# yvette256/nerfstudio-thermal

Hardware: AMD Instinct MI355X
Metric: train rays/sec (4096-ray batch, 96 samples/ray) (higher is better)
Workload: dtype f32; 1 GPU; thermal-nerfacto density_mode=shared train step (pixel sampling+raygen+fwd+losses+bwd+allreduce+Adam), 4096 rays/GPU, 256/96 proposal + 48 field samples, hash 16x2^19x2 + 2x(5x2^17x2), 8 cameras (4 RGB + 4 thermal); rays_per_gpu=4096, parallelism=dp1, grad_scaler=device-side (optim.DeviceGradScaler)

## Files before the change

### nerfstudio-thermal_amd/csrc/tn_common.h

```cpp
#pragma once
#include <hip/hip_runtime.h>
#include <stdint.h>
#include <math.h>
#include "../../include/thermal_nerf_hip.h"

#define TN_WAVE 64

void tn_set_error(const char* fmt, ...);
#define TN_REQUIRE(cond, ...)        \
  do {                               \
    if (!(cond)) {                   \
      tn_set_error(__VA_ARGS__);     \
      return TN_EINVAL;              \
    }                                \
  } while (0)
#define TN_CHECK_LAUNCH(name)                                         \
  do {                                                                \
    hipError_t e__ = hipGetLastError();                               \
    if (e__ != hipSuccess) {                                          \
      tn_set_error("%s: %s", name, hipGetErrorString(e__));           \
      return TN_ELAUNCH;                                              \
    }                                                                 \
  } while (0)

static inline hipStream_t tn_s(tn_stream_t s) { return reinterpret_cast<hipStream_t>(s); }

hipStream_t tn_fork(hipStream_t user);
hipStream_t tn_fork_n(hipStream_t user, int idx);
void tn_join_n(hipStream_t user, int idx);
void tn_join(hipStream_t user, hipStream_t companion);
void tn_join_all(hipStream_t user);
__host__ __device__ static inline int64_t tn_cdiv(int64_t a, int64_t b) { return (a + b - 1) / b; }

struct GridK {
  const float2* table;
  float2* grad;
  int L;
  uint32_t mask;
  uint32_t tsize;
  float res[TN_MAX_LEVELS];
  float* nonfinite;
  int grad_zero;
};
static inline GridK make_gridk(const TnGrid& g) {
  GridK k;
  k.table = reinterpret_cast<const float2*>(g.table);
  k.grad = reinterpret_cast<float2*>(g.table_grad);
  k.L = g.num_levels;
  k.tsize = 1u << g.log2_hashmap_size;
  k.mask = k.tsize - 1u;
  for (int i = 0; i < TN_MAX_LEVELS; ++i) k.res[i] = g.res[i];
  k.nonfinite = g.nonfinite_flag;
  k.grad_zero = g.table_grad_is_zero;
  return k;
}

int tn_prop_density_fwd_ex(const TnPropNet* net, const float* origins, const float* directions, const float* e_bins, int64_t N, int32_t S,
                           float* density, float* enc_out, tn_stream_t stream);
int tn_prop_density_bwd_ex(const TnPropNet* net, const float* origins, const float* directions, const float* e_bins, const float* d_density, int64_t N,
                           int32_t S, void* workspace, int64_t workspace_bytes, float* d_origins, float* d_directions, const float* saved_enc,
                           tn_stream_t stream);
int tn_field_fwd_ex(const TnField* field, const float* origins, const float* directions, const int64_t* camera_indices, const float* e_bins, int64_t N, int32_t S,
                    int32_t training, void* workspace, int64_t workspace_bytes, float* density, float* rgb, float* density_pre, int pack_first, void* zero,
                    int64_t zero_bytes, tn_stream_t stream);

int64_t tn_knn_tree_workspace_bytes(int64_t n);
int tn_knn_neighbor_means(const float* points, int64_t n, int32_t nb_neighbors, double* mean, void* workspace, int64_t workspace_bytes,
                          hipStream_t stream);

struct SplatCropK {
  float m[12];
  float h[3];
};
__device__ __forceinline__ bool splat_in_crop(const SplatCropK& c, float x, float y, float z) {
  bool in = true;
#pragma unroll
  for (int a = 0; a < 3; ++a) {
    const float q = __fadd_rn(__fadd_rn(__fadd_rn(__fmul_rn(c.m[4 * a], x), __fmul_rn(c.m[4 * a + 1], y)), __fmul_rn(c.m[4 * a + 2], z)), c.m[4 * a + 3]);
    in = in && fabsf(q) < c.h[a];
  }
  return in;
}
static inline SplatCropK make_cropk(const TnSplatCrop* crop) {
  SplatCropK c;
  for (int i = 0; i < 12; ++i) c.m[i] = crop->world_to_box[i];
  for (int i = 0; i < 3; ++i) c.h[i] = crop->half_extent[i];
  return c;
}

#define TN_PRIME_Y 2654435761u
#define TN_PRIME_Z 805459861u

__device__ __forceinline__ float tn_nan_to_num(float x) {
  if (x != x) return 0.0f;
  if (x > 3.4028234663852886e38f) return 3.4028234663852886e38f;
  if (x < -3.4028234663852886e38f) return -3.4028234663852886e38f;
  return x;
}

__device__ __forceinline__ float tn_spacing(float x) { return x < 1.0f ? x / 2.0f : 1.0f - 1.0f / (2.0f * x); }
__device__ __forceinline__ float tn_spacing_inv(float x) { return x < 0.5f ? 2.0f * x : 1.0f / (2.0f - 2.0f * x); }
__device__ __forceinline__ float tn_s_to_euclid(float x, float s_near, float s_far) {
  return tn_spacing_inv(x * s_far + (1.0f - x) * s_near);
}

__device__ __forceinline__ int64_t tn_div_index(int64_t i, int64_t d, int64_t total) {
  return total < (1ll << 31) ? (int64_t)((uint32_t)i / (uint32_t)d) : i / d;
}

__device__ __forceinline__ void tn_spaced_bins_ray(const float* __restrict__ lin_bins, bool jittered, float jit, float s_near, float s_far, int S,
                                                   float* __restrict__ sb, float* __restrict__ eb, int lane, float* e_keep = nullptr,
                                                   float* s_keep = nullptr) {
#pragma unroll
  for (int k = 0; k <= TN_MAX_SAMPLES / 64; ++k) {
    const int j = lane + 64 * k;
    if (j > S) continue;
    float b = lin_bins[j];
    if (jittered) {
      float lower = (j == 0) ? lin_bins[0] : (lin_bins[j] + lin_bins[j - 1]) / 2.0f;
      float upper = (j == S) ? lin_bins[S] : (lin_bins[j + 1] + lin_bins[j]) / 2.0f;
      b = lower + (upper - lower) * jit;
    }
    const float e = tn_s_to_euclid(b, s_near, s_far);
    sb[j] = b;
    eb[j] = e;
    if (e_keep != nullptr) e_keep[j] = e;
    if (s_keep != nullptr) s_keep[k] = b;
  }
}
__device__ __forceinline__ void tn_spaced_bins_body(const float* __restrict__ lin_bins, const float* __restrict__ jitter,
                                                    const float* __restrict__ nears, const float* __restrict__ fars, int64_t N, int S,
                                                    float* __restrict__ s_bins, float* __restrict__ e_bins, int bid, int nblk) {
  const int lane = threadIdx.x & 63, wpb = blockDim.x >> 6;
  for (int64_t ray = (int64_t)bid * wpb + (threadIdx.x >> 6); ray < N; ray += (int64_t)nblk * wpb) {
    const float s_near = tn_spacing(nears[ray]), s_far = tn_spacing(fars[ray]);
    const float jit = jitter != nullptr ? jitter[ray] : 0.0f;
    tn_spaced_bins_ray(lin_bins, jitter != nullptr, jit, s_near, s_far, S, s_bins + ray * (S + 1), e_bins + ray * (S + 1), lane);
  }
}

struct Contracted {
  float px, py, pz;
  bool sel;
  float wx, wy, wz;
  float mag;
  int amax;
};
__device__ __forceinline__ Contracted tn_contract(float ox, float oy, float oz, float dx, float dy, float dz, float start, float end) {
  Contracted c;
  float se = start + end;
  c.wx = ox + (dx * se) / 2.0f;
  c.wy = oy + (dy * se) / 2.0f;
  c.wz = oz + (dz * se) / 2.0f;
  float ax = fabsf(c.wx), ay = fabsf(c.wy), az = fabsf(c.wz);
  float mag = fmaxf(fmaxf(ax, ay), az);
  c.mag = mag;
  c.amax = (ax >= ay && ax >= az) ? 0 : (ay >= az ? 1 : 2);
  float x = c.wx, y = c.wy, z = c.wz;
  if (!(mag < 1.0f)) {
    float k = 2.0f - (1.0f / mag);
    x = k * (x / mag);
    y = k * (y / mag);
    z = k * (z / mag);
  }
  x = (x + 2.0f) / 4.0f;
  y = (y + 2.0f) / 4.0f;
  z = (z + 2.0f) / 4.0f;
  c.sel = (x > 0.0f) && (x < 1.0f) && (y > 0.0f) && (y < 1.0f) && (z > 0.0f) && (z < 1.0f);
  float m = c.sel ? 1.0f : 0.0f;
  c.px = x * m;
  c.py = y * m;
  c.pz = z * m;
  return c;
}

__device__ __forceinline__ void tn_contract_bwd(const Contracted& c, float gx, float gy, float gz, float& wx, float& wy, float& wz) {
  if (!c.sel) { wx = wy = wz = 0.0f; return; }
  gx *= 0.25f; gy *= 0.25f; gz *= 0.25f;
  if (c.mag < 1.0f) { wx = gx; wy = gy; wz = gz; return; }
  float m = c.mag;
  float s = 2.0f / m - 1.0f / (m * m);
  float t = (-2.0f / (m * m) + 2.0f / (m * m * m));
  float dot = gx * c.wx + gy * c.wy + gz * c.wz;
  wx = s * gx; wy = s * gy; wz = s * gz;
  float xa = c.amax == 0 ? c.wx : (c.amax == 1 ? c.wy : c.wz);
  float extra = dot * t * (xa >= 0.0f ? 1.0f : -1.0f);
  if (c.amax == 0) wx += extra; else if (c.amax == 1) wy += extra; else wz += extra;
}

struct LevelCorners {
  uint32_t idx[8];
  float ox, oy, oz;
};
__device__ __forceinline__ void tn_level_corners(float px, float py, float pz, float res, uint32_t mask, uint32_t level_off, LevelCorners& lc) {
  float sx = px * res, sy = py * res, sz = pz * res;
  float fxf = floorf(sx), fyf = floorf(sy), fzf = floorf(sz);
  uint32_t cx = (uint32_t)(int)ceilf(sx), cy = (uint32_t)(int)ceilf(sy), cz = (uint32_t)(int)ceilf(sz);
  uint32_t fx = (uint32_t)(int)fxf, fy = (uint32_t)(int)fyf, fz = (uint32_t)(int)fzf;
  lc.ox = sx - fxf; lc.oy = sy - fyf; lc.oz = sz - fzf;
  uint32_t hcy = cy * TN_PRIME_Y, hfy = fy * TN_PRIME_Y, hcz = cz * TN_PRIME_Z, hfz = fz * TN_PRIME_Z;
  lc.idx[0] = ((cx ^ hcy ^ hcz) & mask) + level_off;
  lc.idx[1] = ((cx ^ hfy ^ hcz) & mask) + level_off;
  lc.idx[2] = ((fx ^ hfy ^ hcz) & mask) + level_off;
  lc.idx[3] = ((fx ^ hcy ^ hcz) & mask) + level_off;
  lc.idx[4] = ((cx ^ hcy ^ hfz) & mask) + level_off;
  lc.idx[5] = ((cx ^ hfy ^ hfz) & mask) + level_off;
  lc.idx[6] = ((fx ^ hfy ^ hfz) & mask) + level_off;
  lc.idx[7] = ((fx ^ hcy ^ hfz) & mask) + level_off;
}
// ... 203 lines not shown
```

### nerfstudio-thermal_amd/csrc/tn_pipeline.hip

```cpp
#include "tn_common.h"
#include "tn_pose_finish.h"
#include "tn_adam.h"

namespace {
struct EvalWs {
  float *s0, *e0, *d0, *w0, *s1, *e1, *d1, *w1, *s2, *e2, *w2, *rgb_s, *scratch;
  void* field_ws;
  int64_t bytes;
};
EvalWs eval_layout(void* base, int64_t N, int S0, int S1, int S2, int C) {
  EvalWs w;
  char* p = reinterpret_cast<char*>(base);
  int64_t off = 0;
  auto take = [&](int64_t floats) {
    float* r = reinterpret_cast<float*>(p + off);
    off += ((floats * 4 + 255) / 256) * 256;
    return r;
  };
  w.s0 = take(N * (S0 + 1)); w.e0 = take(N * (S0 + 1)); w.d0 = take(N * S0); w.w0 = take(N * S0);
  w.s1 = take(N * (S1 + 1)); w.e1 = take(N * (S1 + 1)); w.d1 = take(N * S1); w.w1 = take(N * S1);
  w.s2 = take(N * (S2 + 1)); w.e2 = take(N * (S2 + 1)); w.w2 = take(N * S2);
  w.rgb_s = take(N * (int64_t)S2 * C);
  w.scratch = take(TN_RENDER_SCRATCH_FLOATS);
  w.field_ws = p + off;
  off += tn_field_workspace_bytes(N * (int64_t)S2, 0);
  w.bytes = off;
  return w;
}
}

extern "C" int64_t tn_render_rays_eval_workspace_bytes(int64_t num_rays, int32_t S0, int32_t S1, int32_t S2, int32_t C) {
  if (num_rays < 0 || S0 < 1 || S1 < 1 || S2 < 1 || S0 > TN_MAX_SAMPLES || S1 > TN_MAX_SAMPLES || S2 > TN_MAX_SAMPLES || C < 1 || C > 4) return TN_EINVAL;
  return eval_layout(nullptr, num_rays, S0, S1, S2, C).bytes;
}

extern "C" int tn_render_rays_eval(const TnPropNet* prop0, const TnPropNet* prop1, const TnField* field, const float* origins,
                                   const float* directions, const int64_t* camera_indices, const float* nears, const float* fars, int64_t N,
                                   int32_t S0, int32_t S1, int32_t S2, float anneal, const float* lin_spaced0, const float* lin_pdf1,
                                   const float* lin_pdf2, void* workspace, int64_t workspace_bytes, float* rgb, float* accumulation, float* depth_median,
                                   float* depth_expected, float* prop_depth0, float* prop_depth1, float* density, float* e_bins_out,
                                   float* rgb_samples_out, tn_stream_t stream) {
  if (N == 0) return TN_OK;
  TN_REQUIRE(prop0 && prop1 && field && origins && directions && camera_indices && nears && fars && lin_spaced0 && lin_pdf1 && lin_pdf2 &&
                 workspace && rgb && density,
             "tn_render_rays_eval: null pointer");
  TN_REQUIRE(N > 0 && S0 >= 1 && S1 >= 1 && S2 >= 1 && S0 <= TN_MAX_SAMPLES && S1 <= TN_MAX_SAMPLES && S2 <= TN_MAX_SAMPLES,
             "tn_render_rays_eval: bad N=%lld S=(%d, %d, %d)", (long long)N, S0, S1, S2);
  TN_REQUIRE(((uintptr_t)workspace % 256) == 0, "tn_render_rays_eval: workspace must be 256-byte aligned");
  const int C = field->num_channels;
  EvalWs w = eval_layout(workspace, N, S0, S1, S2, C);
  TN_REQUIRE(workspace_bytes >= w.bytes, "tn_render_rays_eval: workspace of %lld bytes, tn_render_rays_eval_workspace_bytes = %lld", (long long)workspace_bytes,
             (long long)w.bytes);
  const int64_t field_ws_bytes = tn_field_workspace_bytes(N * (int64_t)S2, 0);
  float* e2 = e_bins_out ? e_bins_out : w.e2;
  float* rgb_s = rgb_samples_out ? rgb_samples_out : w.rgb_s;
  int rc;
  if ((rc = tn_spaced_bins(lin_spaced0, nullptr, nears, fars, N, S0, w.s0, w.e0, stream))) return rc;
  if ((rc = tn_prop_density_fwd(prop0, origins, directions, w.e0, N, S0, w.d0, stream))) return rc;
  if ((rc = tn_weights_resample(w.e0, w.d0, w.s0, S0, anneal, lin_pdf1, nullptr, nears, fars, N, S1, w.w0, prop_depth0, w.s1, w.e1, stream))) return rc;
  if ((rc = tn_prop_density_fwd(prop1, origins, directions, w.e1, N, S1, w.d1, stream))) return rc;
  if ((rc = tn_weights_resample(w.e1, w.d1, w.s1, S1, anneal, lin_pdf2, nullptr, nears, fars, N, S2, w.w1, prop_depth1, w.s2, e2, stream))) return rc;
  if ((rc = tn_field_fwd_ex(field, origins, directions, camera_indices, e2, N, S2, 0, w.field_ws, field_ws_bytes, density, rgb_s, nullptr, 1, nullptr, 0, stream)))
    return rc;
  return tn_render_fwd(e2, density, rgb_s, N, S2, C, 0, w.w2, rgb, accumulation, depth_median, depth_expected, w.scratch, stream);
}

enum {
  TRO_ORIGINS = 0, TRO_DIRECTIONS,
  TRO_S0, TRO_E0, TRO_D0, TRO_W0, TRO_M0,
  TRO_S1, TRO_E1, TRO_D1, TRO_W1, TRO_M1,
  TRO_S2, TRO_E2, TRO_D2, TRO_W2,
  TRO_RGB_SAMPLES, TRO_COMP, TRO_ACC, TRO_DEPTH, TRO_EXPECTED, TRO_SCRATCH,
  TRO_PENC0, TRO_PENC1,
  TRO_END,
  TRO_COUNT
};
static void train_layout(int64_t N, int S0, int S1, int S2, int C, int64_t* off) {
  int64_t o = 0;
  auto take = [&](int slot, int64_t floats) { off[slot] = o; o += (floats + 63) / 64 * 64; };
  take(TRO_ORIGINS, N * 3); take(TRO_DIRECTIONS, N * 3);
  take(TRO_S0, N * (S0 + 1)); take(TRO_E0, N * (S0 + 1)); take(TRO_D0, N * S0); take(TRO_W0, N * S0); take(TRO_M0, N);
  take(TRO_S1, N * (S1 + 1)); take(TRO_E1, N * (S1 + 1)); take(TRO_D1, N * S1); take(TRO_W1, N * S1); take(TRO_M1, N);
  take(TRO_S2, N * (S2 + 1)); take(TRO_E2, N * (S2 + 1)); take(TRO_D2, N * S2); take(TRO_W2, N * S2);
  take(TRO_RGB_SAMPLES, N * (int64_t)S2 * C); take(TRO_COMP, N * C); take(TRO_ACC, N); take(TRO_DEPTH, N); take(TRO_EXPECTED, N);
  take(TRO_SCRATCH, TN_RENDER_SCRATCH_FLOATS);
  take(TRO_PENC0, N * (int64_t)S0 * 10); take(TRO_PENC1, N * (int64_t)S1 * 10);
  off[TRO_END] = o;
}

extern "C" int tn_render_rays_train_layout(int64_t num_rays, int32_t S0, int32_t S1, int32_t S2, int32_t C, int64_t* offsets, int32_t num_offsets) {
  TN_REQUIRE(offsets != nullptr && num_offsets >= TRO_COUNT, "tn_render_rays_train_layout: offsets needs %d entries", (int)TRO_COUNT);
  TN_REQUIRE(num_rays >= 0 && S0 >= 1 && S1 >= 1 && S2 >= 1 && S0 <= TN_MAX_SAMPLES && S1 <= TN_MAX_SAMPLES && S2 <= TN_MAX_SAMPLES && C >= 1 && C <= 4,
             "tn_render_rays_train_layout: bad argument");
  train_layout(num_rays, S0, S1, S2, C, offsets);
  return TN_OK;
}

static int render_rays_train_impl(const TnPropNet* prop0, const TnPropNet* prop1, const TnField* field, const float* pose_adjustment,
                                  const uint8_t* frozen, int32_t num_cameras, const float* origins_in, const float* directions_in,
                                  const int64_t* camera_indices, const float* nears, const float* fars, int64_t N, int32_t S0, int32_t S1,
                                  int32_t S2, float anneal, const float* jitter0, const float* jitter1, const float* jitter2,
                                  const float* lin_spaced0, const float* lin_pdf1, const float* lin_pdf2, void* field_workspace,
                                  int64_t field_workspace_bytes, float* out, void* wait_event_before_field, void* zero_fill, int64_t zero_fill_bytes,
                                  int32_t save_prop_enc, int with_render, int* clip_nblk, tn_stream_t stream, bool sampling_done = false) {
  if (clip_nblk) *clip_nblk = 0;
  if (N == 0) return TN_OK;
  TN_REQUIRE(prop0 && prop1 && field && origins_in && directions_in && camera_indices && nears && fars && lin_spaced0 && lin_pdf1 && lin_pdf2 &&
                 field_workspace && out,
             "tn_render_rays_train: null pointer");
  TN_REQUIRE(N > 0 && S0 >= 1 && S1 >= 1 && S2 >= 1 && S0 <= TN_MAX_SAMPLES && S1 <= TN_MAX_SAMPLES && S2 <= TN_MAX_SAMPLES,
             "tn_render_rays_train: bad N=%lld S=(%d, %d, %d)", (long long)N, S0, S1, S2);
  TN_REQUIRE(((uintptr_t)out % 256) == 0, "tn_render_rays_train: the output buffer must be 256-byte aligned");
  const int C = field->num_channels;
  int64_t off[TRO_COUNT];
  train_layout(N, S0, S1, S2, C, off);
  auto at = [&](int slot) { return out + off[slot]; };
  const float* o = origins_in;
  const float* d = directions_in;
  int rc;
  if (sampling_done) {
    if (pose_adjustment != nullptr) { o = at(TRO_ORIGINS); d = at(TRO_DIRECTIONS); }
  } else {
    if (pose_adjustment != nullptr) {
      TN_REQUIRE(num_cameras >= 1, "tn_render_rays_train: bad num_cameras=%d", num_cameras);
      if ((rc = tn_pose_spaced_bins(pose_adjustment, frozen, camera_indices, origins_in, directions_in, N, num_cameras, at(TRO_ORIGINS), at(TRO_DIRECTIONS),
                                    lin_spaced0, jitter0, nears, fars, S0, at(TRO_S0), at(TRO_E0), stream)))
        return rc;
      o = at(TRO_ORIGINS);
      d = at(TRO_DIRECTIONS);
    } else if ((rc = tn_spaced_bins(lin_spaced0, jitter0, nears, fars, N, S0, at(TRO_S0), at(TRO_E0), stream))) {
      return rc;
    }
    if ((rc = tn_prop_density_fwd_ex(prop0, o, d, at(TRO_E0), N, S0, at(TRO_D0), save_prop_enc ? at(TRO_PENC0) : nullptr, stream))) return rc;
    if ((rc = tn_weights_resample(at(TRO_E0), at(TRO_D0), at(TRO_S0), S0, anneal, lin_pdf1, jitter1, nears, fars, N, S1, at(TRO_W0), at(TRO_M0), at(TRO_S1),
                                  at(TRO_E1), stream)))
      return rc;
    if ((rc = tn_prop_density_fwd_ex(prop1, o, d, at(TRO_E1), N, S1, at(TRO_D1), save_prop_enc ? at(TRO_PENC1) : nullptr, stream))) return rc;
    if ((rc = tn_weights_resample(at(TRO_E1), at(TRO_D1), at(TRO_S1), S1, anneal, lin_pdf2, jitter2, nears, fars, N, S2, at(TRO_W1), at(TRO_M1), at(TRO_S2),
                                  at(TRO_E2), stream)))
      return rc;
  }
  if (wait_event_before_field != nullptr) {
    hipError_t e = hipStreamWaitEvent(tn_s(stream), reinterpret_cast<hipEvent_t>(wait_event_before_field), 0);
    TN_REQUIRE(e == hipSuccess, "tn_render_rays_train: hipStreamWaitEvent failed: %s", hipGetErrorString(e));
  }
  if ((rc = tn_field_fwd_ex(field, o, d, camera_indices, at(TRO_E2), N, S2, 1, field_workspace, field_workspace_bytes, at(TRO_D2), at(TRO_RGB_SAMPLES), nullptr, 1,
                            zero_fill, zero_fill_bytes, stream)))
    return rc;
  if (!with_render) return TN_OK;
  return tn_render_fwd_ex(at(TRO_E2), at(TRO_D2), at(TRO_RGB_SAMPLES), N, S2, C, 1, at(TRO_W2), at(TRO_COMP), at(TRO_ACC), at(TRO_DEPTH), at(TRO_EXPECTED),
                          at(TRO_SCRATCH), with_render == 1, clip_nblk, stream);
}
extern "C" int tn_render_rays_train(const TnPropNet* prop0, const TnPropNet* prop1, const TnField* field, const float* pose_adjustment,
                                    const uint8_t* frozen, int32_t num_cameras, const float* origins_in, const float* directions_in,
                                    const int64_t* camera_indices, const float* nears, const float* fars, int64_t N, int32_t S0, int32_t S1,
                                    int32_t S2, float anneal, const float* jitter0, const float* jitter1, const float* jitter2,
                                    const float* lin_spaced0, const float* lin_pdf1, const float* lin_pdf2, void* field_workspace,
                                    int64_t field_workspace_bytes, float* out, void* wait_event_before_field, void* zero_fill, int64_t zero_fill_bytes,
                                    int32_t save_prop_enc, tn_stream_t stream) {
  return render_rays_train_impl(prop0, prop1, field, pose_adjustment, frozen, num_cameras, origins_in, directions_in, camera_indices, nears, fars, N, S0, S1, S2,
                                anneal, jitter0, jitter1, jitter2, lin_spaced0, lin_pdf1, lin_pdf2, field_workspace, field_workspace_bytes, out,
                                wait_event_before_field, zero_fill, zero_fill_bytes, save_prop_enc, 1, nullptr, stream);
}

__global__ void k_add_inplace(float* __restrict__ a, const float* __restrict__ b, int64_t n) {
  for (int64_t i = blockIdx.x * (int64_t)blockDim.x + threadIdx.x; i < n; i += (int64_t)gridDim.x * blockDim.x) a[i] += b[i];
}
extern "C" int64_t tn_render_rays_train_bwd_tmp_floats(int64_t N, int32_t S0, int32_t S1, int32_t S2, int32_t C) {
  if (N < 0 || S0 < 1 || S1 < 1 || S2 < 1 || C < 1 || C > 4) return TN_EINVAL;
  auto up = [](int64_t x) { return (x + 63) / 64 * 64; };
  return up(N * (int64_t)S2 * C) + up(N * (int64_t)S2) + up(N * (int64_t)S0) + up(N * (int64_t)S1);
}
static int render_rays_train_bwd_impl(const TnPropNet* prop0, const TnPropNet* prop1, const TnField* field, const float* origins,
                                      const float* directions, const int64_t* camera_indices, int64_t N, int32_t S0, int32_t S1, int32_t S2,
                                      const float* fwd_out, const float* d_comp, const float* d_weights0,
                                      const float* d_weights1, const float* d_weights2, const float* d_density_extra, void* field_workspace,
                                      int64_t field_workspace_bytes, void* prop_workspace0, int64_t prop_workspace_bytes0, void* prop_workspace1,
                                      int64_t prop_workspace_bytes1, float* tmp, float* d_origins, float* d_directions, int32_t prop_enc_saved,
                                      bool render_bwd_done, const PoseFinishArgs* fold_cowork, bool* fold_cowork_taken, tn_stream_t stream,
                                      const FoldAdamHost* fold_adam = nullptr) {
  if (fold_cowork_taken) *fold_cowork_taken = false;
  if (N == 0) return TN_OK;
  TN_REQUIRE(field && origins && directions && camera_indices && fwd_out && d_comp && d_weights2 && field_workspace && tmp,
             "tn_render_rays_train_bwd: null pointer");
  TN_REQUIRE((d_weights0 == nullptr) == (d_weights1 == nullptr), "tn_render_rays_train_bwd: d_weights0 and d_weights1 come together (or not at all)");
  const bool prop_grad = d_weights0 != nullptr;
  if (prop_grad) TN_REQUIRE(prop0 && prop1 && prop_workspace0 && prop_workspace1, "tn_render_rays_train_bwd: proposal networks / workspaces missing");
  TN_REQUIRE(N > 0 && S0 >= 1 && S1 >= 1 && S2 >= 1 && S0 <= TN_MAX_SAMPLES && S1 <= TN_MAX_SAMPLES && S2 <= TN_MAX_SAMPLES,
             "tn_render_rays_train_bwd: bad N=%lld S=(%d, %d, %d)", (long long)N, S0, S1, S2);
  TN_REQUIRE((d_origins == nullptr) == (d_directions == nullptr), "tn_render_rays_train_bwd: d_origins and d_directions must both be given or both NULL");
  const int C = field->num_channels;
  int64_t off[TRO_COUNT];
  train_layout(N, S0, S1, S2, C, off);
  auto at = [&](int slot) { return fwd_out + off[slot]; };
  auto up = [](int64_t x) { return (x + 63) / 64 * 64; };
  float* d_rgb = tmp;
  float* d_dens = d_rgb + up(N * (int64_t)S2 * C);
  float* dd0 = d_dens + up(N * (int64_t)S2);
  float* dd1 = dd0 + up(N * (int64_t)S0);
  const float* o = origins;
  const float* d = directions;
  hipStream_t st = tn_s(stream);
  int rc;
  if (!render_bwd_done && (rc = tn_render_bwd(at(TRO_E2), at(TRO_D2), at(TRO_RGB_SAMPLES), at(TRO_W2), d_comp, d_weights2, N, S2, C, d_rgb, d_dens, stream)))
    return rc;
  if (d_density_extra != nullptr) {
    const int64_t n = N * (int64_t)S2;
    hipLaunchKernelGGL(k_add_inplace, dim3((unsigned)std::min<int64_t>(tn_cdiv(n, 256), 4096)), dim3(256), 0, st, d_dens, d_density_extra, n);
    TN_CHECK_LAUNCH("tn_render_rays_train_bwd(add)");
  }
  int rc0 = TN_OK, rc1 = TN_OK;
  if (prop_grad) {
    hipStream_t s0 = tn_fork_n(st, 1), s1 = tn_fork_n(st, 2);
    tn_stream_t t0 = s0 ? (tn_stream_t)s0 : stream, t1 = s1 ? (tn_stream_t)s1 : stream;
    rc0 = tn_weights_bwd(at(TRO_E0), at(TRO_D0), at(TRO_W0), d_weights0, N, S0, dd0, t0);
    if (!rc0)
      rc0 = tn_prop_density_bwd_ex(prop0, o, d, at(TRO_E0), dd0, N, S0, prop_workspace0, prop_workspace_bytes0, d_origins, d_directions,
                                   prop_enc_saved ? at(TRO_PENC0) : nullptr, t0);
    rc1 = tn_weights_bwd(at(TRO_E1), at(TRO_D1), at(TRO_W1), d_weights1, N, S1, dd1, t1);
    if (!rc1)
      rc1 = tn_prop_density_bwd_ex(prop1, o, d, at(TRO_E1), dd1, N, S1, prop_workspace1, prop_workspace_bytes1, d_origins, d_directions,
                                   prop_enc_saved ? at(TRO_PENC1) : nullptr, t1);
  }
  rc = tn_field_bwd_phase_ex(field, o, d, camera_indices, at(TRO_E2), d_dens, d_rgb, N, S2, field_workspace, field_workspace_bytes, d_origins, d_directions,
                             TN_BWD_MLP | TN_BWD_SCATTER | TN_BWD_JOIN | (prop_grad ? TN_BWD_FORK_DPOS : 0), 0, field->grid.num_levels,
                             prop_grad ? nullptr : fold_cowork, fold_cowork_taken, stream, fold_adam);
  if (prop_grad) { tn_join_n(st, 1); tn_join_n(st, 2); }
  return rc ? rc : (rc0 ? rc0 : rc1);
}
extern "C" int tn_render_rays_train_bwd(const TnPropNet* prop0, const TnPropNet* prop1, const TnField* field, const float* origins,
                                        const float* directions, const int64_t* camera_indices, int64_t N, int32_t S0, int32_t S1, int32_t S2,
                                        const float* fwd_out, const float* d_comp, const float* d_weights0,
                                        const float* d_weights1, const float* d_weights2, const float* d_density_extra, void* field_workspace,
                                        int64_t field_workspace_bytes, void* prop_workspace0, int64_t prop_workspace_bytes0, void* prop_workspace1,
                                        int64_t prop_workspace_bytes1, float* tmp, float* d_origins, float* d_directions, int32_t prop_enc_saved,
                                        tn_stream_t stream) {
  return render_rays_train_bwd_impl(prop0, prop1, field, origins, directions, camera_indices, N, S0, S1, S2, fwd_out, d_comp, d_weights0, d_weights1, d_weights2,
                                    d_density_extra, field_workspace, field_workspace_bytes, prop_workspace0, prop_workspace_bytes0, prop_workspace1,
                                    prop_workspace_bytes1, tmp, d_origins, d_directions, prop_enc_saved, false, nullptr, nullptr, stream);
// ... 237 lines not shown
```

### nerfstudio-thermal_amd/csrc/tn_prop.hip

```cpp
#include "tn_common.h"
#include "tn_prop_point.h"

template <bool SAVE_ENC>
__global__ void __launch_bounds__(256, 2) k_prop_fwd(PropK net, const float* __restrict__ origins, const float* __restrict__ directions,
                                                     const float* __restrict__ e_bins, int64_t N, int S, float* __restrict__ density,
                                                     float* __restrict__ enc_out) {
  __shared__ __attribute__((aligned(16))) float s_w[PH * PROP_WROW + 4];
  prop_stage_weights(net, s_w);
  int64_t P = N * (int64_t)S;
  for (int64_t i = blockIdx.x * (int64_t)blockDim.x + threadIdx.x; i < P; i += (int64_t)gridDim.x * blockDim.x) {
    int64_t ray = tn_div_index(i, S, P);
    int s = (int)(i - ray * S);
    const float* o = origins + ray * 3;
    const float* d = directions + ray * 3;
    const float* eb = e_bins + ray * (S + 1) + s;
    Contracted c = tn_contract(o[0], o[1], o[2], d[0], d[1], d[2], eb[0], eb[1]);
    float enc[PF];
#pragma unroll
    for (int l = 0; l < PL; ++l) {
      float2 v = tn_encode_level(net.g.table, c.px, c.py, c.pz, net.g.res[l], net.g.mask, (uint32_t)l * net.g.tsize);
      enc[2 * l] = v.x;
      enc[2 * l + 1] = v.y;
      if (SAVE_ENC) *reinterpret_cast<float2*>(enc_out + ((int64_t)l * P + i) * 2) = v;
    }
    const float out = prop_mlp(s_w, enc);
    density[i] = c.sel ? expf(out) : 0.0f * expf(out);
  }
}

extern "C" int tn_prop_density_fwd(const TnPropNet* net, const float* origins, const float* directions, const float* e_bins, int64_t N,
                                   int32_t S, float* density, tn_stream_t stream) {
  return tn_prop_density_fwd_ex(net, origins, directions, e_bins, N, S, density, nullptr, stream);
}
int tn_prop_density_fwd_ex(const TnPropNet* net, const float* origins, const float* directions, const float* e_bins, int64_t N, int32_t S,
                           float* density, float* enc_out, tn_stream_t stream) {
  if (N == 0) return TN_OK;
  TN_REQUIRE(net && origins && directions && e_bins && density, "tn_prop_density_fwd: null pointer");
  TN_REQUIRE(net->grid.table && net->w0 && net->b0 && net->w1 && net->b1, "tn_prop_density_fwd: null parameter pointer");
  TN_REQUIRE(net->grid.num_levels == PL, "tn_prop_density_fwd: proposal grids are built for %d levels, got %d", PL, net->grid.num_levels);
  TN_REQUIRE(net->grid.log2_hashmap_size >= 1 && net->grid.log2_hashmap_size <= 24, "tn_prop_density_fwd: bad log2_hashmap_size");
  TN_REQUIRE(N >= 0 && S >= 1 && S <= TN_MAX_SAMPLES, "tn_prop_density_fwd: bad N=%lld S=%d", (long long)N, S);
  if (N == 0) return TN_OK;
  PropK k{make_gridk(net->grid), net->w0, net->b0, net->w1, net->b1, nullptr, nullptr, nullptr, nullptr};
  int64_t P = N * (int64_t)S;
  int grid = (int)std::min<int64_t>(tn_cdiv(P, 256), 256 * 16);
  if (enc_out != nullptr)
    hipLaunchKernelGGL(k_prop_fwd<true>, dim3(grid), dim3(256), 0, tn_s(stream), k, origins, directions, e_bins, N, S, density, enc_out);
  else
    hipLaunchKernelGGL(k_prop_fwd<false>, dim3(grid), dim3(256), 0, tn_s(stream), k, origins, directions, e_bins, N, S, density, enc_out);
  TN_CHECK_LAUNCH("tn_prop_density_fwd");
  return TN_OK;
}

typedef float f32x4_t __attribute__((ext_vector_type(4)));

#define PB_RS 12
#define PB_RS2 16
#define PB_WAVE_FLOATS (64 * PB_RS + 64 * PB_RS2 + 64)
#define PB_WAVE_SYNC()                                    \
  do {                                                    \
    __builtin_amdgcn_fence(__ATOMIC_RELEASE, "wavefront"); \
    __builtin_amdgcn_wave_barrier();                      \
    __builtin_amdgcn_fence(__ATOMIC_ACQUIRE, "wavefront"); \
  } while (0)

__device__ __forceinline__ float prop_row_sum(float x) {
  x += __builtin_bit_cast(float, __builtin_amdgcn_update_dpp(0, __builtin_bit_cast(int, x), 0xB1, 0xf, 0xf, false));
  x += __builtin_bit_cast(float, __builtin_amdgcn_update_dpp(0, __builtin_bit_cast(int, x), 0x4E, 0xf, 0xf, false));
  x += __builtin_bit_cast(float, __builtin_amdgcn_update_dpp(0, __builtin_bit_cast(int, x), 0x141, 0xf, 0xf, false));
  x += __builtin_bit_cast(float, __builtin_amdgcn_update_dpp(0, __builtin_bit_cast(int, x), 0x140, 0xf, 0xf, false));
  return x;
}

#define PB_THREADS 1024
template <bool HAVE_ENC>
__global__ void __launch_bounds__(PB_THREADS) k_prop_bwd_mlp(PropK net, const float* __restrict__ origins, const float* __restrict__ directions,
                                                               const float* __restrict__ e_bins, const float* __restrict__ d_density, int64_t N, int S,
                                                               float* __restrict__ ws_denc, uint32_t* __restrict__ zero_ptr, int zero_words,
                                                               const float* __restrict__ saved_enc) {
  __shared__ __attribute__((aligned(16))) float lds[(PB_THREADS / 64) * PB_WAVE_FLOATS];
  tn_zero_words(zero_ptr, zero_words);
  const int lane = threadIdx.x & 63, wv = threadIdx.x >> 6;
  const int g = lane >> 4, n = lane & 15;
  float* E = lds + wv * PB_WAVE_FLOATS;
  float* DA = E + 64 * PB_RS;
  float* DD = DA + 64 * PB_RS2;
  float wf[3], wb[4], w1q[4];
#pragma unroll
  for (int t = 0; t < 3; ++t) {
    const int f = 4 * t + g;
    wf[t] = f < PF ? net.w0[n * PF + f] : (f == PF ? net.b0[n] : 0.0f);
  }
#pragma unroll
  for (int r = 0; r < 4; ++r) {
    wb[r] = n < PF ? net.w0[(4 * g + r) * PF + n] : 0.0f;
    w1q[r] = net.w1[4 * g + r];
  }
  const float b1 = net.b1[0];
  int64_t P = N * (int64_t)S;
  f32x4_t G[2] = {{0.f, 0.f, 0.f, 0.f}, {0.f, 0.f, 0.f, 0.f}};
  float dw1[4] = {0.f, 0.f, 0.f, 0.f}, sum_dout = 0.0f;
  float n_enc[PF], n_dd = 0.0f;
  const int64_t stride = (int64_t)gridDim.x * blockDim.x;
  auto fetch = [&](int64_t b0) {
    const int64_t i = b0 + lane;
    const bool live = i < P;
    const int64_t ic = live ? i : P - 1;
    int64_t ray = tn_div_index(ic, S, P);
    int s = (int)(ic - ray * S);
    const float* o = origins + ray * 3;
    const float* d = directions + ray * 3;
    const float* eb = e_bins + ray * (S + 1) + s;
    Contracted c = tn_contract(o[0], o[1], o[2], d[0], d[1], d[2], eb[0], eb[1]);
    n_dd = (live && c.sel) ? d_density[ic] : 0.0f;
#pragma unroll
    for (int l = 0; l < PL; ++l) {
      const float2 v = HAVE_ENC ? *reinterpret_cast<const float2*>(saved_enc + ((int64_t)l * P + ic) * 2)
                                : tn_encode_level(net.g.table, c.px, c.py, c.pz, net.g.res[l], net.g.mask, (uint32_t)l * net.g.tsize);
      n_enc[2 * l] = v.x;
      n_enc[2 * l + 1] = v.y;
    }
  };
  int64_t base = (blockIdx.x * (int64_t)(blockDim.x >> 6) + wv) * 64;
  if (base < P) fetch(base);
  for (; base < P; base += stride) {
    *reinterpret_cast<float4*>(E + lane * PB_RS + 0) = make_float4(n_enc[0], n_enc[1], n_enc[2], n_enc[3]);
    *reinterpret_cast<float4*>(E + lane * PB_RS + 4) = make_float4(n_enc[4], n_enc[5], n_enc[6], n_enc[7]);
    *reinterpret_cast<float4*>(E + lane * PB_RS + 8) = make_float4(n_enc[8], n_enc[9], 1.0f, 0.0f);
    DD[lane] = n_dd;
    if (base + stride < P) fetch(base + stride);
    PB_WAVE_SYNC();
#pragma unroll
    for (int h = 0; h < 2; ++h) {
      f32x4_t T[2] = {{0.f, 0.f, 0.f, 0.f}, {0.f, 0.f, 0.f, 0.f}};
#pragma unroll
      for (int t = 0; t < 3; ++t)
#pragma unroll
        for (int q = 0; q < 2; ++q)
          T[q] = __builtin_amdgcn_mfma_f32_16x16x4f32(wf[t], E[(16 * (2 * h + q) + n) * PB_RS + 4 * t + g], T[q], 0, 0, 0);
      float part[2];
#pragma unroll
      for (int q = 0; q < 2; ++q) {
        part[q] = 0.0f;
#pragma unroll
        for (int r = 0; r < 4; ++r) part[q] = fmaf(w1q[r], fmaxf(T[q][r], 0.0f), part[q]);
      }
#pragma unroll
      for (int q = 0; q < 2; ++q) part[q] += __shfl_xor(part[q], 16, 64);
#pragma unroll
      for (int q = 0; q < 2; ++q) part[q] += __shfl_xor(part[q], 32, 64);
      f32x4_t X[2] = {{0.f, 0.f, 0.f, 0.f}, {0.f, 0.f, 0.f, 0.f}};
      float da[2][4];
#pragma unroll
      for (int q = 0; q < 2; ++q) {
        const int c = 2 * h + q;
        const float d_out = DD[16 * c + n] * expf(fminf(fmaxf(b1 + part[q], -15.0f), 15.0f));
        if (g == 0) sum_dout += d_out;
#pragma unroll
        for (int r = 0; r < 4; ++r) {
          dw1[r] = fmaf(d_out, fmaxf(T[q][r], 0.0f), dw1[r]);
          da[q][r] = T[q][r] > 0.0f ? d_out * w1q[r] : 0.0f;
        }
      }
#pragma unroll
      for (int r = 0; r < 4; ++r)
#pragma unroll
        for (int q = 0; q < 2; ++q) X[q] = __builtin_amdgcn_mfma_f32_16x16x4f32(wb[r], da[q][r], X[q], 0, 0, 0);
#pragma unroll
      for (int q = 0; q < 2; ++q) {
        const int c = 2 * h + q;
        *reinterpret_cast<float4*>(DA + (16 * c + n) * PB_RS2 + 4 * g) = make_float4(da[q][0], da[q][1], da[q][2], da[q][3]);
        const int64_t is = base + 16 * c + n;
        if (is < P && g < 3) {
          *reinterpret_cast<float2*>(ws_denc + ((int64_t)(2 * g) * P + is) * 2) = make_float2(X[q][0], X[q][1]);
          if (g < 2) *reinterpret_cast<float2*>(ws_denc + ((int64_t)(2 * g + 1) * P + is) * 2) = make_float2(X[q][2], X[q][3]);
        }
      }
    }
    PB_WAVE_SYNC();
#pragma unroll
    for (int t = 0; t < 16; ++t) {
      const float e = n < PB_RS ? E[(4 * t + g) * PB_RS + n] : 0.0f;
      G[t & 1] = __builtin_amdgcn_mfma_f32_16x16x4f32(e, DA[(4 * t + g) * PB_RS2 + n], G[t & 1], 0, 0, 0);
    }
    PB_WAVE_SYNC();
  }
#pragma unroll
  for (int r = 0; r < 4; ++r) G[0][r] = G[0][r] + G[1][r];
#pragma unroll
  for (int r = 0; r < 4; ++r) dw1[r] = prop_row_sum(dw1[r]);
  sum_dout = tn_wave_sum(sum_dout);
  {
    float* mine = E;
#pragma unroll
    for (int r = 0; r < 4; ++r) mine[(4 * g + r) * 16 + n] = G[0][r];
    if (n == 0) {
#pragma unroll
      for (int r = 0; r < 4; ++r) mine[256 + 4 * g + r] = dw1[r];
    }
    if (lane == 0) mine[272] = sum_dout;
  }
  __syncthreads();
  if (threadIdx.x < 273) {
    float v = 0.0f;
#pragma unroll
    for (int w = 0; w < PB_THREADS / 64; ++w) v += lds[w * PB_WAVE_FLOATS + threadIdx.x];
    const int f = threadIdx.x >> 4, h = threadIdx.x & 15;
    if (v != 0.0f) {
      if (f < PF) atomicAdd(net.gw0 + h * PF + f, v);
      else if (f == PF) atomicAdd(net.gb0 + h, v);
      else if (f == 16) atomicAdd(net.gw1 + h, v);
      else if (threadIdx.x == 272) atomicAdd(net.gb1, v);
    }
  }
}

static inline int64_t prop_scratch_offset(int64_t P) { return ((P * 16 * (int64_t)sizeof(float) + 1024 + 255) / 256) * 256; }

extern "C" int64_t tn_prop_workspace_bytes(int64_t num_points) {
  if (num_points < 0) return TN_EINVAL;
  return prop_scratch_offset(num_points) + tn_scatter_scratch_bytes(num_points, PL);
}

extern "C" int tn_prop_density_bwd(const TnPropNet* net, const float* origins, const float* directions, const float* e_bins,
                                   const float* d_density, int64_t N, int32_t S, void* workspace, int64_t workspace_bytes, float* d_origins,
                                   float* d_directions, tn_stream_t stream) {
  return tn_prop_density_bwd_ex(net, origins, directions, e_bins, d_density, N, S, workspace, workspace_bytes, d_origins, d_directions, nullptr, stream);
}
int tn_prop_density_bwd_ex(const TnPropNet* net, const float* origins, const float* directions, const float* e_bins, const float* d_density, int64_t N,
                           int32_t S, void* workspace, int64_t workspace_bytes, float* d_origins, float* d_directions, const float* saved_enc,
                           tn_stream_t stream) {
  if (N == 0) return TN_OK;
  TN_REQUIRE(net && origins && directions && e_bins && d_density && workspace, "tn_prop_density_bwd: null pointer");
  TN_REQUIRE(net->grid.table && net->grid.table_grad && net->w0 && net->b0 && net->w1 && net->b1 && net->gw0 && net->gb0 && net->gw1 && net->gb1,
             "tn_prop_density_bwd: null parameter/gradient pointer");
  TN_REQUIRE((d_origins == nullptr) == (d_directions == nullptr), "tn_prop_density_bwd: d_origins and d_directions must both be given or both NULL");
  TN_REQUIRE(net->grid.num_levels == PL, "tn_prop_density_bwd: proposal grids are built for %d levels, got %d", PL, net->grid.num_levels);
  TN_REQUIRE(net->grid.log2_hashmap_size >= 1 && net->grid.log2_hashmap_size <= 24, "tn_prop_density_bwd: bad log2_hashmap_size");
  TN_REQUIRE(N >= 0 && S >= 1 && S <= TN_MAX_SAMPLES, "tn_prop_density_bwd: bad N=%lld S=%d", (long long)N, S);
  TN_REQUIRE(((uintptr_t)workspace % 256) == 0, "tn_prop_density_bwd: workspace must be 256-byte aligned");
  TN_REQUIRE(workspace_bytes >= tn_prop_workspace_bytes(N * (int64_t)S), "tn_prop_density_bwd: workspace of %lld bytes, tn_prop_workspace_bytes(%lld) = %lld",
             (long long)workspace_bytes, (long long)(N * (int64_t)S), (long long)tn_prop_workspace_bytes(N * (int64_t)S));
  if (N == 0) return TN_OK;
  PropK k{make_gridk(net->grid), net->w0, net->b0, net->w1, net->b1, net->gw0, net->gb0, net->gw1, net->gb1};
  int64_t P = N * (int64_t)S;
  float* ws_denc = reinterpret_cast<float*>(workspace);
  int grid = (int)std::min<int64_t>(tn_cdiv(P, PB_THREADS), 256);
  const int threads = PB_THREADS;
  hipStream_t st = tn_s(stream);
  void* scratch = reinterpret_cast<char*>(workspace) + prop_scratch_offset(P);
  uint32_t* zp;
  int zw;
  tn_grid_scatter_counters(net->grid, P, scratch, &zp, &zw);
  if (saved_enc != nullptr)
    hipLaunchKernelGGL(k_prop_bwd_mlp<true>, dim3(grid), dim3(threads), 0, st, k, origins, directions, e_bins, d_density, N, S, ws_denc, zp, zw, saved_enc);
  else
    hipLaunchKernelGGL(k_prop_bwd_mlp<false>, dim3(grid), dim3(threads), 0, st, k, origins, directions, e_bins, d_density, N, S, ws_denc, zp, zw, saved_enc);
  TN_CHECK_LAUNCH("tn_prop_density_bwd");
  return tn_grid_scatter_launch(net->grid, origins, directions, e_bins, ws_denc, TN_LD_LEVEL_MAJOR, N, S, d_origins, d_directions, scratch, st, nullptr,
                                zw > 0);
}
```

### nerfstudio-thermal_amd/csrc/tn_prop_point.h

```cpp
#pragma once
#include "tn_common.h"

#define PL 5
#define PF 10
#define PH 16
#define PROP_NW (PH * PF + PH + PH + 1)

struct PropK {
  GridK g;
  const float *w0, *b0, *w1, *b1;
  float *gw0, *gb0, *gw1, *gb1;
};

#define PROP_WROW 12
__device__ __forceinline__ int prop_weight_slot(int j, int k) { return (j >> 1) * (2 * PROP_WROW) + 2 * k + (j & 1); }
__device__ __forceinline__ void prop_stage_weights_into(const float* __restrict__ w0, const float* __restrict__ b0, const float* __restrict__ w1,
                                                        const float* __restrict__ b1, float* s_w) {
  for (int t = threadIdx.x; t < PH * PROP_WROW; t += blockDim.x) {
    const int j = t / PROP_WROW, k = t - j * PROP_WROW;
    s_w[prop_weight_slot(j, k)] = k < PF ? w0[j * PF + k] : (k == PF ? b0[j] : w1[j]);
  }
  if (threadIdx.x == 0) s_w[PH * PROP_WROW] = b1[0];
}
__device__ __forceinline__ void prop_stage_weights(const PropK& net, float* s_w) {
  prop_stage_weights_into(net.w0, net.b0, net.w1, net.b1, s_w);
  __syncthreads();
}
__device__ __forceinline__ float prop_mlp(const float* s_w, const float (&enc)[PF]) {
  float out = s_w[PH * PROP_WROW];
#pragma unroll 2
  for (int q = 0; q < PH / 2; ++q) {
    const float4* row = reinterpret_cast<const float4*>(s_w + q * 2 * PROP_WROW);
    const float4 r0 = row[0], r1 = row[1], r2 = row[2], r3 = row[3], r4 = row[4], r5 = row[5];
    tn_v2f a = {r5.x, r5.y};
    a = __builtin_elementwise_fma(tn_v2f{r0.x, r0.y}, tn_v2f{enc[0], enc[0]}, a);
    a = __builtin_elementwise_fma(tn_v2f{r0.z, r0.w}, tn_v2f{enc[1], enc[1]}, a);
    a = __builtin_elementwise_fma(tn_v2f{r1.x, r1.y}, tn_v2f{enc[2], enc[2]}, a);
    a = __builtin_elementwise_fma(tn_v2f{r1.z, r1.w}, tn_v2f{enc[3], enc[3]}, a);
    a = __builtin_elementwise_fma(tn_v2f{r2.x, r2.y}, tn_v2f{enc[4], enc[4]}, a);
    a = __builtin_elementwise_fma(tn_v2f{r2.z, r2.w}, tn_v2f{enc[5], enc[5]}, a);
    a = __builtin_elementwise_fma(tn_v2f{r3.x, r3.y}, tn_v2f{enc[6], enc[6]}, a);
    a = __builtin_elementwise_fma(tn_v2f{r3.z, r3.w}, tn_v2f{enc[7], enc[7]}, a);
    a = __builtin_elementwise_fma(tn_v2f{r4.x, r4.y}, tn_v2f{enc[8], enc[8]}, a);
    a = __builtin_elementwise_fma(tn_v2f{r4.z, r4.w}, tn_v2f{enc[9], enc[9]}, a);
    out = fmaf(r5.z, fmaxf(a.x, 0.0f), out);
    out = fmaf(r5.w, fmaxf(a.y, 0.0f), out);
  }
  return out;
}

struct PropNoHook { __device__ __forceinline__ void operator()() const {} };
template <bool SAVE_ENC, bool LEVEL_FENCE = false, bool OPTIONAL_ENC = false, class Hook = PropNoHook>
__device__ __forceinline__ float prop_density_sample(const PropK& net, const float* s_w, float px, float py, float pz, bool sel, int64_t i, int64_t P, float* enc_out,
                                                     Hook hook = Hook()) {
  float enc[PF];
#pragma unroll
  for (int l = 0; l < PL; ++l) {
    if (LEVEL_FENCE && l > 0) __builtin_amdgcn_sched_barrier(0);
    float2 v = tn_encode_level(net.g.table, px, py, pz, net.g.res[l], net.g.mask, (uint32_t)l * net.g.tsize);
    enc[2 * l] = v.x;
    enc[2 * l + 1] = v.y;
    if (__is_same(Hook, PropNoHook) && SAVE_ENC && (!OPTIONAL_ENC || enc_out != nullptr)) *reinterpret_cast<float2*>(enc_out + ((int64_t)l * P + i) * 2) = v;
  }
  if (!__is_same(Hook, PropNoHook)) {
    asm volatile("" :: "v"(enc[0]), "v"(enc[1]), "v"(enc[2]), "v"(enc[3]), "v"(enc[4]), "v"(enc[5]), "v"(enc[6]), "v"(enc[7]), "v"(enc[8]), "v"(enc[9]));
    hook();
    if (SAVE_ENC && (!OPTIONAL_ENC || enc_out != nullptr)) {
#pragma unroll
      for (int l = 0; l < PL; ++l) *reinterpret_cast<float2*>(enc_out + ((int64_t)l * P + i) * 2) = make_float2(enc[2 * l], enc[2 * l + 1]);
    }
  }
  const float out = prop_mlp(s_w, enc);
  return sel ? expf(out) : 0.0f * expf(out);
}
```

Baseline: 6.103 million rays/s.

## Add MFMA-based proposal MLP backward with block partial reduction and saved selection mask

Replaces the proposal-network MLP backward kernel with a version that runs the 16-wide hidden layer's forward recompute, input-gradient, and weight-gradient products on MFMA 16x16x4 f32 instructions, one wave per 64 samples. It software-prefetches the next chunk's encodings and writes per-block weight-gradient partials to a workspace, which a small finish kernel sums after the grid scatter. The forward now also saves a per-sample selection byte next to the saved encodings, so the backward skips re-running ray contraction when encodings are available. The cost is a larger saved-encoding buffer, an extra kernel launch, and a new env-gated code path.

```diff
diff --git a/nerfstudio-thermal_amd/csrc/tn_common.h b/nerfstudio-thermal_amd/csrc/tn_common.h
--- a/nerfstudio-thermal_amd/csrc/tn_common.h
+++ b/nerfstudio-thermal_amd/csrc/tn_common.h
@@ -55,6 +55,9 @@
   return k;
 }
 
+static inline int64_t tn_prop_saved_enc_floats(int64_t P) { return P * 10 + (P + 3) / 4; }
+__host__ __device__ __forceinline__ uint8_t* prop_saved_sel(float* enc_out, int64_t P) { return reinterpret_cast<uint8_t*>(enc_out + P * 10); }
+__host__ __device__ __forceinline__ const uint8_t* prop_saved_sel(const float* enc_out, int64_t P) { return reinterpret_cast<const uint8_t*>(enc_out + P * 10); }
 int tn_prop_density_fwd_ex(const TnPropNet* net, const float* origins, const float* directions, const float* e_bins, int64_t N, int32_t S,
                            float* density, float* enc_out, tn_stream_t stream);
 int tn_prop_density_bwd_ex(const TnPropNet* net, const float* origins, const float* directions, const float* e_bins, const float* d_density, int64_t N,
diff --git a/nerfstudio-thermal_amd/csrc/tn_pipeline.hip b/nerfstudio-thermal_amd/csrc/tn_pipeline.hip
--- a/nerfstudio-thermal_amd/csrc/tn_pipeline.hip
+++ b/nerfstudio-thermal_amd/csrc/tn_pipeline.hip
@@ -84,7 +84,7 @@
   take(TRO_S2, N * (S2 + 1)); take(TRO_E2, N * (S2 + 1)); take(TRO_D2, N * S2); take(TRO_W2, N * S2);
   take(TRO_RGB_SAMPLES, N * (int64_t)S2 * C); take(TRO_COMP, N * C); take(TRO_ACC, N); take(TRO_DEPTH, N); take(TRO_EXPECTED, N);
   take(TRO_SCRATCH, TN_RENDER_SCRATCH_FLOATS);
-  take(TRO_PENC0, N * (int64_t)S0 * 10); take(TRO_PENC1, N * (int64_t)S1 * 10);
+  take(TRO_PENC0, tn_prop_saved_enc_floats(N * (int64_t)S0)); take(TRO_PENC1, tn_prop_saved_enc_floats(N * (int64_t)S1));
   off[TRO_END] = o;
 }
 
diff --git a/nerfstudio-thermal_amd/csrc/tn_prop.hip b/nerfstudio-thermal_amd/csrc/tn_prop.hip
--- a/nerfstudio-thermal_amd/csrc/tn_prop.hip
+++ b/nerfstudio-thermal_amd/csrc/tn_prop.hip
@@ -23,6 +23,7 @@
       enc[2 * l + 1] = v.y;
       if (SAVE_ENC) *reinterpret_cast<float2*>(enc_out + ((int64_t)l * P + i) * 2) = v;
     }
+    if (SAVE_ENC) prop_saved_sel(enc_out, P)[i] = c.sel ? 1 : 0;
     const float out = prop_mlp(s_w, enc);
     density[i] = c.sel ? expf(out) : 0.0f * expf(out);
   }
@@ -215,7 +216,203 @@
   }
 }
 
-static inline int64_t prop_scratch_offset(int64_t P) { return ((P * 16 * (int64_t)sizeof(float) + 1024 + 255) / 256) * 256; }
+#define PB2_THREADS 256
+#define PB2_MAX_BLOCKS 1024
+#define PB2_PART_STRIDE 288
+template <bool HAVE_ENC>
+__global__ void __launch_bounds__(PB2_THREADS, 4) k_prop_bwd_mlp2(PropK net, const float* __restrict__ origins, const float* __restrict__ directions,
+                                                                  const float* __restrict__ e_bins, const float* __restrict__ d_density, int64_t N, int S,
+                                                                  float* __restrict__ ws_denc, uint32_t* __restrict__ zero_ptr, int zero_words,
+                                                                  const float* __restrict__ saved_enc, float* __restrict__ ws_part) {
+  __shared__ __attribute__((aligned(16))) float lds[(PB2_THREADS / 64) * PB_WAVE_FLOATS];
+  tn_zero_words(zero_ptr, zero_words);
+  const int lane = threadIdx.x & 63, wv = threadIdx.x >> 6;
+  const int g = lane >> 4, n = lane & 15;
+  float* E = lds + wv * PB_WAVE_FLOATS;
+  float* DA = E + 64 * PB_RS;
+  float* DD = DA + 64 * PB_RS2;
+  float wf[3], wb[4], w1q[4];
+#pragma unroll
+  for (int t = 0; t < 3; ++t) {
+    const int f = 4 * t + g;
+    wf[t] = f < PF ? net.w0[n * PF + f] : (f == PF ? net.b0[n] : 0.0f);
+  }
+#pragma unroll
+  for (int r = 0; r < 4; ++r) {
+    wb[r] = n < PF ? net.w0[(4 * g + r) * PF + n] : 0.0f;
+    w1q[r] = net.w1[4 * g + r];
+  }
+  const float b1 = net.b1[0];
+  const int64_t P = N * (int64_t)S;
+  f32x4_t G[2] = {{0.f, 0.f, 0.f, 0.f}, {0.f, 0.f, 0.f, 0.f}};
+  float dw1[4] = {0.f, 0.f, 0.f, 0.f}, sum_dout = 0.0f;
+  float n_enc[PF], n_dd = 0.0f;
+  const uint8_t* __restrict__ saved_sel = HAVE_ENC ? prop_saved_sel(saved_enc, P) : nullptr;
+  const int64_t stride = (int64_t)gridDim.x * blockDim.x;
+  auto fetch = [&](int64_t b0, float (&enc)[PF], float& dd) {
+    const int64_t i = b0 + lane;
+    const bool live = i < P;
+    const int64_t ic = live ? i : P - 1;
+    if (HAVE_ENC) {
+      const float dv = d_density[ic];
+      const uint8_t sel = saved_sel[ic];
+#pragma unroll
+      for (int l = 0; l < PL; ++l) {
+        const float2 v = *reinterpret_cast<const float2*>(saved_enc + ((int64_t)l * P + ic) * 2);
+        enc[2 * l] = v.x;
+        enc[2 * l + 1] = v.y;
+      }
+      dd = (live && sel != 0) ? dv : 0.0f;
+    } else {
+      int64_t ray = tn_div_index(ic, S, P);
+      int s = (int)(ic - ray * S);
+      const float* o = origins + ray * 3;
+      const float* d = directions + ray * 3;
+      const float* eb = e_bins + ray * (S + 1) + s;
+      Contracted c = tn_contract(o[0], o[1], o[2], d[0], d[1], d[2], eb[0], eb[1]);
+      dd = (live && c.sel) ? d_density[ic] : 0.0f;
+#pragma unroll
+      for (int l = 0; l < PL; ++l) {
+        const float2 v = tn_encode_level(net.g.table, c.px, c.py, c.pz, net.g.res[l], net.g.mask, (uint32_t)l * net.g.tsize);
+        enc[2 * l] = v.x;
+        enc[2 * l + 1] = v.y;
+      }
+    }
+  };
+  int64_t base = (blockIdx.x * (int64_t)(PB2_THREADS / 64) + wv) * 64;
+  if (base < P) fetch(base, n_enc, n_dd);
+  for (; base < P; base += stride) {
+    float (&enc)[PF] = n_enc;
+    float& dd = n_dd;
+    *reinterpret_cast<float4*>(E + lane * PB_RS + 0) = make_float4(enc[0], enc[1], enc[2], enc[3]);
+    *reinterpret_cast<float4*>(E + lane * PB_RS + 4) = make_float4(enc[4], enc[5], enc[6], enc[7]);
+    *reinterpret_cast<float4*>(E + lane * PB_RS + 8) = make_float4(enc[8], enc[9], 1.0f, 0.0f);
+    DD[lane] = dd;
+    if (base + stride < P) fetch(base + stride, enc, dd);
+    PB_WAVE_SYNC();
+#pragma unroll
+    for (int h = 0; h < 2; ++h) {
+      f32x4_t T[2] = {{0.f, 0.f, 0.f, 0.f}, {0.f, 0.f, 0.f, 0.f}};
+#pragma unroll
+      for (int t = 0; t < 3; ++t)
+#pragma unroll
+        for (int q = 0; q < 2; ++q)
+          T[q] = __builtin_amdgcn_mfma_f32_16x16x4f32(wf[t], E[(16 * (2 * h + q) + n) * PB_RS + 4 * t + g], T[q], 0, 0, 0);
+      float part[2];
+#pragma unroll
+      for (int q = 0; q < 2; ++q) {
+        part[q] = 0.0f;
+#pragma unroll
+        for (int r = 0; r < 4; ++r) part[q] = fmaf(w1q[r], fmaxf(T[q][r], 0.0f), part[q]);
+      }
+#pragma unroll
+      for (int q = 0; q < 2; ++q) part[q] += __shfl_xor(part[q], 16, 64);
+#pragma unroll
+      for (int q = 0; q < 2; ++q) part[q] += __shfl_xor(part[q], 32, 64);
+      f32x4_t X[2] = {{0.f, 0.f, 0.f, 0.f}, {0.f, 0.f, 0.f, 0.f}};
+      float da[2][4];
+#pragma unroll
+      for (int q = 0; q < 2; ++q) {
+        const int c = 2 * h + q;
+        const float d_out = DD[16 * c + n] * expf(fminf(fmaxf(b1 + part[q], -15.0f), 15.0f));
+        if (g == 0) sum_dout += d_out;
+#pragma unroll
+        for (int r = 0; r < 4; ++r) {
+          dw1[r] = fmaf(d_out, fmaxf(T[q][r], 0.0f), dw1[r]);
+          da[q][r] = T[q][r] > 0.0f ? d_out * w1q[r] : 0.0f;
+        }
+      }
+#pragma unroll
+      for (int r = 0; r < 4; ++r)
+#pragma unroll
+        for (int q = 0; q < 2; ++q) X[q] = __builtin_amdgcn_mfma_f32_16x16x4f32(wb[r], da[q][r], X[q], 0, 0, 0);
+#pragma unroll
+      for (int q = 0; q < 2; ++q) {
+        const int c = 2 * h + q;
+        *reinterpret_cast<float4*>(DA + (16 * c + n) * PB_RS2 + 4 * g) = make_float4(da[q][0], da[q][1], da[q][2], da[q][3]);
+        const int64_t is = base + 16 * c + n;
+        if (is < P && g < 3) {
+          *reinterpret_cast<float2*>(ws_denc + ((int64_t)(2 * g) * P + is) * 2) = make_float2(X[q][0], X[q][1]);
+          if (g < 2) *reinterpret_cast<float2*>(ws_denc + ((int64_t)(2 * g + 1) * P + is) * 2) = make_float2(X[q][2], X[q][3]);
+        }
+      }
+    }
+    PB_WAVE_SYNC();
+#pragma unroll
+    for (int t = 0; t < 16; ++t) {
+      const float e = n < PB_RS ? E[(4 * t + g) * PB_RS + n] : 0.0f;
+      G[t & 1] = __builtin_amdgcn_mfma_f32_16x16x4f32(e, DA[(4 * t + g) * PB_RS2 + n], G[t & 1], 0, 0, 0);
+    }
+    PB_WAVE_SYNC();
+  }
+#pragma unroll
+  for (int r = 0; r < 4; ++r) G[0][r] = G[0][r] + G[1][r];
+#pragma unroll
+  for (int r = 0; r < 4; ++r) dw1[r] = prop_row_sum(dw1[r]);
+  sum_dout = tn_wave_sum(sum_dout);
+  {
+    float* mine = E;
+#pragma unroll
+    for (int r = 0; r < 4; ++r) mine[(4 * g + r) * 16 + n] = G[0][r];
+    if (n == 0) {
+#pragma unroll
+      for (int r = 0; r < 4; ++r) mine[256 + 4 * g + r] = dw1[r];
+    }
+    if (lane == 0) mine[272] = sum_dout;
+  }
+  __syncthreads();
+  for (int t = threadIdx.x; t < 273; t += PB2_THREADS) {
+    float v = 0.0f;
+#pragma unroll
+    for (int w = 0; w < PB2_THREADS / 64; ++w) v += lds[w * PB_WAVE_FLOATS + t];
+    ws_part[(int64_t)blockIdx.x * PB2_PART_STRIDE + t] = v;
+  }
+}
+
+#define PBF_THREADS 1024
+__global__ void __launch_bounds__(PBF_THREADS) k_prop_bwd_finish(const float* __restrict__ ws_part, int nblk, float* __restrict__ gw0, float* __restrict__ gb0,
+                                                                  float* __restrict__ gw1, float* __restrict__ gb1) {
+  __shared__ float s_sum[PBF_THREADS / 64][64];
+  const int lane = threadIdx.x & 63, wv = threadIdx.x >> 6;
+  const int t = blockIdx.x * 64 + lane;
+  float v = 0.0f;
+  if (t < 273) {
+#pragma unroll 8
+    for (int b = wv; b < nblk; b += PBF_THREADS / 64) v += ws_part[(int64_t)b * PB2_PART_STRIDE + t];
+  }
+  s_sum[wv][lane] = v;
+  __syncthreads();
+  if (wv == 0 && t < 273) {
+    v = 0.0f;
+#pragma unroll
+    for (int w = 0; w < PBF_THREADS / 64; ++w) v += s_sum[w][lane];
+    const int f = t >> 4, h = t & 15;
+    if (f < PF) gw0[h * PF + f] += v;
+    else if (f == PF) gb0[h] += v;
+    else if (f == 16) gw1[h] += v;
+    else if (t == 272) gb1[0] += v;
+  }
+}
+
+static bool prop_bwd_mlp2_on() {
+  static const bool on = [] { const char* e = getenv("TN_PROP_BWD"); return !(e && e[0] == '0'); }();
+  return on;
+}
+static int prop_bwd_max_blocks() {
+  static const int nb = [] {
+    const char* e = getenv("TN_PROP_BWD_BLOCKS");
+    const int v = e ? atoi(e) : 0;
+    return v >= 1 && v <= PB2_MAX_BLOCKS ? v : PB2_MAX_BLOCKS;
+  }();
+  return nb;
+}
+static inline int prop_bwd_blocks(int64_t P) { return (int)std::min<int64_t>(tn_cdiv(P, PB2_THREADS), prop_bwd_max_blocks()); }
+
+static inline int64_t prop_part_offset(int64_t P) { return ((P * 16 * (int64_t)sizeof(float) + 1024 + 255) / 256) * 256; }
+static inline int64_t prop_scratch_offset(int64_t P) {
+  const int64_t nblk = std::min<int64_t>(tn_cdiv(P, PB2_THREADS), PB2_MAX_BLOCKS);
+  return prop_part_offset(P) + ((nblk * PB2_PART_STRIDE * (int64_t)sizeof(float) + 255) / 256) * 256;
+}
 
 extern "C" int64_t tn_prop_workspace_bytes(int64_t num_points) {
   if (num_points < 0) return TN_EINVAL;
@@ -252,11 +449,28 @@
   uint32_t* zp;
   int zw;
   tn_grid_scatter_counters(net->grid, P, scratch, &zp, &zw);
-  if (saved_enc != nullptr)
-    hipLaunchKernelGGL(k_prop_bwd_mlp<true>, dim3(grid), dim3(threads), 0, st, k, origins, directions, e_bins, d_density, N, S, ws_denc, zp, zw, saved_enc);
-  else
-    hipLaunchKernelGGL(k_prop_bwd_mlp<false>, dim3(grid), dim3(threads), 0, st, k, origins, directions, e_bins, d_density, N, S, ws_denc, zp, zw, saved_enc);
-  TN_CHECK_LAUNCH("tn_prop_density_bwd");
+  if (prop_bwd_mlp2_on()) {
+    float* ws_part = reinterpret_cast<float*>(reinterpret_cast<char*>(workspace) + prop_part_offset(P));
+    const int nblk = prop_bwd_blocks(P);
+    if (saved_enc != nullptr)
+      hipLaunchKernelGGL(k_prop_bwd_mlp2<true>, dim3(nblk), dim3(PB2_THREADS), 0, st, k, origins, directions, e_bins, d_density, N, S, ws_denc, zp, zw, saved_enc,
+                         ws_part);
+    else
+      hipLaunchKernelGGL(k_prop_bwd_mlp2<false>, dim3(nblk), dim3(PB2_THREADS), 0, st, k, origins, directions, e_bins, d_density, N, S, ws_denc, zp, zw, saved_enc,
+                         ws_part);
+    TN_CHECK_LAUNCH("tn_prop_density_bwd");
+    int rc = tn_grid_scatter_launch(net->grid, origins, directions, e_bins, ws_denc, TN_LD_LEVEL_MAJOR, N, S, d_origins, d_directions, scratch, st, nullptr, zw > 0);
+    if (rc) return rc;
+    hipLaunchKernelGGL(k_prop_bwd_finish, dim3(tn_cdiv(273, 64)), dim3(PBF_THREADS), 0, st, ws_part, nblk, k.gw0, k.gb0, k.gw1, k.gb1);
+    TN_CHECK_LAUNCH("tn_prop_density_bwd(finish)");
+    return TN_OK;
+  } else {
+    if (saved_enc != nullptr)
+      hipLaunchKernelGGL(k_prop_bwd_mlp<true>, dim3(grid), dim3(threads), 0, st, k, origins, directions, e_bins, d_density, N, S, ws_denc, zp, zw, saved_enc);
+    else
+      hipLaunchKernelGGL(k_prop_bwd_mlp<false>, dim3(grid), dim3(threads), 0, st, k, origins, directions, e_bins, d_density, N, S, ws_denc, zp, zw, saved_enc);
+    TN_CHECK_LAUNCH("tn_prop_density_bwd");
+  }
   return tn_grid_scatter_launch(net->grid, origins, directions, e_bins, ws_denc, TN_LD_LEVEL_MAJOR, N, S, d_origins, d_directions, scratch, st, nullptr,
                                 zw > 0);
 }
diff --git a/nerfstudio-thermal_amd/csrc/tn_prop_point.h b/nerfstudio-thermal_amd/csrc/tn_prop_point.h
--- a/nerfstudio-thermal_amd/csrc/tn_prop_point.h
+++ b/nerfstudio-thermal_amd/csrc/tn_prop_point.h
@@ -70,6 +70,7 @@
       for (int l = 0; l < PL; ++l) *reinterpret_cast<float2*>(enc_out + ((int64_t)l * P + i) * 2) = make_float2(enc[2 * l], enc[2 * l + 1]);
     }
   }
+  if (SAVE_ENC && (!OPTIONAL_ENC || enc_out != nullptr)) prop_saved_sel(enc_out, P)[i] = sel ? 1 : 0;
   const float out = prop_mlp(s_w, enc);
   return sel ? expf(out) : 0.0f * expf(out);
 }
```

New measurement: 6.145 million rays/s, median of 6. No clear change (+0.7%).
